# SLIDE-3D/SLIDE

Hardware: AMD Instinct MI355X
Metric: latent shapes/sec (pos+feat DDPM, 1000 steps, 16 pts) (higher is better)
Workload: dtype f16 (MFMA operands + activation storage; f32 accumulate, norm statistics, softmax); position DDPM: two-term f16 operand splits (fp32-grade); 1 GPU; BASELINE configs[1]+[2]: airplane position DDPM (16x3) + chair feature DDPM (16x51), batch 256 per GPU; 1 step = one reverse step of each; shape = 1000+1000 steps; batch_per_gpu=256, prec=fp16, pos_prec=split, replay=eager, pos_batch_multiple=2, pos_stream_cus=176, prime_steps=0, finite=True

## Files before the change

### slide_amd/csrc/gemm_ring.hip

```cpp
#include "gemm_common.h"
#include "gemm_small.h"
#include "launch.h"

namespace {

template <int PREC, int NPXL, int CBW, bool PAIRRES = false>
__global__ __launch_bounds__(256, (PREC == SLIDE_PREC_SPLIT && NPXL == 4) ? 1 : 2) void gemm_kernel(GemmArgs a) {
  using T = typename TileT<PREC>::T;
  constexpr int LDK = TileT<PREC>::LDK;
  constexpr int EPL = TileT<PREC>::EPL;
  constexpr int TPR = BK / EPL;
  constexpr int RPP = 256 / TPR;
  constexpr int TN = 32 * CBW;
  constexpr int XP = TM / RPP, WP = TN / RPP;
  extern __shared__ __attribute__((aligned(16))) unsigned char smem_raw[];
  constexpr bool SPLIT = PREC == SLIDE_PREC_SPLIT;
  using TS = typename std::conditional<SPLIT, _Float16, T>::type;
  TS *const sbase = reinterpret_cast<TS *>(smem_raw);
  constexpr int STAGE = (SPLIT ? 2 : 1) * (TM + TN) * LDK;
  constexpr int NSTG = SPLIT ? 1 : 2;
  constexpr bool AFF_LDS = PREC != SLIDE_PREC_F16 && NPXL >= 7;
  constexpr int AFF_NS = TM >> (NPXL >= 7 ? NPXL : 7);

  const int ntc = (a.n_cob + CBW - 1) / CBW;
  const int ntr = (a.rows + TM - 1) / TM;
  const int xcd = blockIdx.x & 7, q0 = blockIdx.x >> 3;
  const int tc = q0 % ntc, tr = (q0 / ntc) * 8 + xcd;
  if (tr >= ntr) return;
  const int row0 = tr * TM, cob0 = tc * CBW;
  const int tid = threadIdx.x, lane = tid & 63, wave = tid >> 6;
  const int half = lane >> 5, col = lane & 31;
  const T *X = reinterpret_cast<const T *>(a.X);
  const T *W = reinterpret_cast<const T *>(a.W);

  f32x16 acc[CBW][2];
  f32x16 acc2[SPLIT ? CBW : 1][2];
#pragma unroll
  for (int i = 0; i < CBW; ++i)
#pragma unroll
    for (int j = 0; j < 2; ++j)
#pragma unroll
      for (int r = 0; r < 16; ++r) {
        acc[i][j][r] = 0.f;
        if (SPLIT) acc2[SPLIT ? i : 0][j][r] = 0.f;
      }

  float4 xr[XP], wr[WP];
  const int l_row = tid / TPR, l_c = (tid % TPR) * EPL;

  auto load_chunk = [&](int kc) {
#pragma unroll
    for (int p = 0; p < XP; ++p) {
      const int grow = row0 + p * RPP + l_row;
      float4 v = make_float4(0.f, 0.f, 0.f, 0.f);
      if (grow < a.rows) {
        v = *reinterpret_cast<const float4 *>(X + (size_t)grow * a.x_ld + kc * BK + l_c);
        if (a.in_scale && !AFF_LDS) {
          const size_t o = (size_t)(grow >> NPXL) * a.in_bs + kc * BK + l_c;
          if (PREC != SLIDE_PREC_F16) {
            const float4 sc = *reinterpret_cast<const float4 *>(a.in_scale + o);
            const float4 sh = *reinterpret_cast<const float4 *>(a.in_shift + o);
            v.x = v.x * sc.x + sh.x; v.y = v.y * sc.y + sh.y; v.z = v.z * sc.z + sh.z; v.w = v.w * sc.w + sh.w;
          } else {
            f16x8 h = *reinterpret_cast<f16x8 *>(&v);
#pragma unroll
            for (int j = 0; j < 8; ++j) h[j] = (_Float16)((float)h[j] * a.in_scale[o + j] + a.in_shift[o + j]);
            v = *reinterpret_cast<float4 *>(&h);
          }
        }
      }
      xr[p] = v;
    }
#pragma unroll
    for (int p = 0; p < WP; ++p) {
      const int gco = cob0 * 32 + p * RPP + l_row;
      wr[p] = gco < a.n_cob * 32 ? *reinterpret_cast<const float4 *>(W + (size_t)gco * a.k_pad + kc * BK + l_c)
                                 : make_float4(0.f, 0.f, 0.f, 0.f);
    }
  };
  const float *aff_lds = nullptr;
  auto store_chunk = [&](int s, int kc) {
    TS *Xs = sbase + s * STAGE;
    TS *Ws = Xs + TM * LDK;
    if constexpr (AFF_LDS) {
      if (a.in_scale) {
#pragma unroll
        for (int p = 0; p < XP; ++p) {
          const int trow = p * RPP + l_row;
          if (row0 + trow < a.rows) {
            const float *ap = aff_lds + (size_t)((trow >> NPXL) * 2) * a.k_pad + kc * BK + l_c;
            const float4 sc = *reinterpret_cast<const float4 *>(ap), sh = *reinterpret_cast<const float4 *>(ap + a.k_pad);
            float4 &v = xr[p];
            v.x = v.x * sc.x + sh.x; v.y = v.y * sc.y + sh.y; v.z = v.z * sc.z + sh.z; v.w = v.w * sc.w + sh.w;
          }
        }
      }
    }
    if constexpr (SPLIT) {
      _Float16 *Xl = Xs + (TM + TN) * LDK, *Wl = Xl + TM * LDK;
#pragma unroll
      for (int p = 0; p < XP; ++p) {
        f16x4 hi, lo;
        split4(xr[p], hi, lo);
        *reinterpret_cast<f16x4 *>(Xs + (p * RPP + l_row) * LDK + l_c) = hi;
        *reinterpret_cast<f16x4 *>(Xl + (p * RPP + l_row) * LDK + l_c) = lo;
      }
#pragma unroll
      for (int p = 0; p < WP; ++p) {
        f16x4 hi, lo;
        split4(wr[p], hi, lo);
        *reinterpret_cast<f16x4 *>(Ws + (p * RPP + l_row) * LDK + l_c) = hi;
        *reinterpret_cast<f16x4 *>(Wl + (p * RPP + l_row) * LDK + l_c) = lo;
      }
    } else {
#pragma unroll
      for (int p = 0; p < XP; ++p) *reinterpret_cast<float4 *>(Xs + (p * RPP + l_row) * LDK + l_c) = xr[p];
#pragma unroll
      for (int p = 0; p < WP; ++p) *reinterpret_cast<float4 *>(Ws + (p * RPP + l_row) * LDK + l_c) = wr[p];
    }
  };
  auto compute = [&](int s) {
    const TS *Xs = sbase + s * STAGE;
    const TS *Ws = Xs + TM * LDK;
    if constexpr (SPLIT) {
      const _Float16 *Xl = Xs + (TM + TN) * LDK, *Wl = Xl + TM * LDK;
#pragma unroll
      for (int st = 0; st < 2; ++st) {
        f16x8 ah[CBW], al[CBW], bh[2], bl[2];
#pragma unroll
        for (int cb = 0; cb < CBW; ++cb) {
          ah[cb] = *reinterpret_cast<const f16x8 *>(Ws + (cb * 32 + col) * LDK + st * 16 + half * 8);
          al[cb] = *reinterpret_cast<const f16x8 *>(Wl + (cb * 32 + col) * LDK + st * 16 + half * 8);
        }
#pragma unroll
        for (int rb = 0; rb < 2; ++rb) {
          bh[rb] = *reinterpret_cast<const f16x8 *>(Xs + (wave * 64 + rb * 32 + col) * LDK + st * 16 + half * 8);
          bl[rb] = *reinterpret_cast<const f16x8 *>(Xl + (wave * 64 + rb * 32 + col) * LDK + st * 16 + half * 8);
        }
#pragma unroll
        for (int cb = 0; cb < CBW; ++cb)
#pragma unroll
          for (int rb = 0; rb < 2; ++rb) {
            acc[cb][rb] = __builtin_amdgcn_mfma_f32_32x32x16_f16(ah[cb], bh[rb], acc[cb][rb], 0, 0, 0);
            acc2[SPLIT ? cb : 0][rb] = __builtin_amdgcn_mfma_f32_32x32x16_f16(ah[cb], bl[rb], acc2[SPLIT ? cb : 0][rb], 0, 0, 0);
            acc2[SPLIT ? cb : 0][rb] = __builtin_amdgcn_mfma_f32_32x32x16_f16(al[cb], bh[rb], acc2[SPLIT ? cb : 0][rb], 0, 0, 0);
          }
      }
    } else if (PREC == SLIDE_PREC_F32) {
      const float *Xf = reinterpret_cast<const float *>(Xs);
      const float *Wf = reinterpret_cast<const float *>(Ws);
#pragma unroll
      for (int q = 0; q < 4; ++q) {
        float4 af[CBW], bf[2];
#pragma unroll
        for (int cb = 0; cb < CBW; ++cb)
          af[cb] = *reinterpret_cast<const float4 *>(Wf + (cb * 32 + col) * LDK + q * 8 + half * 4);
#pragma unroll
        for (int rb = 0; rb < 2; ++rb)
          bf[rb] = *reinterpret_cast<const float4 *>(Xf + (wave * 64 + rb * 32 + col) * LDK + q * 8 + half * 4);
#pragma unroll
        for (int cb = 0; cb < CBW; ++cb)
#pragma unroll
          for (int rb = 0; rb < 2; ++rb) {
            acc[cb][rb] = __builtin_amdgcn_mfma_f32_32x32x2f32(af[cb].x, bf[rb].x, acc[cb][rb], 0, 0, 0);
            acc[cb][rb] = __builtin_amdgcn_mfma_f32_32x32x2f32(af[cb].y, bf[rb].y, acc[cb][rb], 0, 0, 0);
            acc[cb][rb] = __builtin_amdgcn_mfma_f32_32x32x2f32(af[cb].z, bf[rb].z, acc[cb][rb], 0, 0, 0);
            acc[cb][rb] = __builtin_amdgcn_mfma_f32_32x32x2f32(af[cb].w, bf[rb].w, acc[cb][rb], 0, 0, 0);
          }
      }
    } else {
      const _Float16 *Xh = reinterpret_cast<const _Float16 *>(Xs);
      const _Float16 *Wh = reinterpret_cast<const _Float16 *>(Ws);
#pragma unroll
      for (int st = 0; st < 2; ++st) {
        f16x8 af[CBW], bf[2];
#pragma unroll
        for (int cb = 0; cb < CBW; ++cb)
          af[cb] = *reinterpret_cast<const f16x8 *>(Wh + (cb * 32 + col) * LDK + st * 16 + half * 8);
#pragma unroll
        for (int rb = 0; rb < 2; ++rb)
          bf[rb] = *reinterpret_cast<const f16x8 *>(Xh + (wave * 64 + rb * 32 + col) * LDK + st * 16 + half * 8);
#pragma unroll
        for (int cb = 0; cb < CBW; ++cb)
#pragma unroll
          for (int rb = 0; rb < 2; ++rb)
            acc[cb][rb] = __builtin_amdgcn_mfma_f32_32x32x16_f16(af[cb], bf[rb], acc[cb][rb], 0, 0, 0);
      }
    }
  };

  uint32_t *const epi_lds = reinterpret_cast<uint32_t *>(smem_raw + NSTG * (size_t)STAGE * sizeof(TS));
  float *const vec_lds = reinterpret_cast<float *>(epi_lds + CBW * EPI_DW + (CBW * EPI_DW) % 4);
  stage_epilogue_tables<CBW>(a, cob0, tid, epi_lds, vec_lds);
  if constexpr (AFF_LDS) {
    if (a.in_scale) {
      float *al = vec_lds + CBW * 96;
      const int nb = a.rows >> NPXL;
      for (int i = tid * 4; i < AFF_NS * a.k_pad; i += 1024) {
        const int sm = i / a.k_pad, k = i - sm * a.k_pad;
        int b = (row0 >> NPXL) + sm;
        b = b < nb ? b : nb - 1;
        *reinterpret_cast<float4 *>(al + (size_t)(sm * 2 + 0) * a.k_pad + k) = *reinterpret_cast<const float4 *>(a.in_scale + (size_t)b * a.in_bs + k);
        *reinterpret_cast<float4 *>(al + (size_t)(sm * 2 + 1) * a.k_pad + k) = *reinterpret_cast<const float4 *>(a.in_shift + (size_t)b * a.in_bs + k);
      }
      aff_lds = al;
      __syncthreads();
    }
  }

  const int nk = a.k_pad / BK;
#ifdef SLIDE_STAGGER
  const int koff = (tc * 5 + tr * 3) % nk;
#define KIDX(k) (((k) + koff) % nk)
#else
#define KIDX(k) (k)
#endif
  load_chunk(KIDX(0));
  store_chunk(0, KIDX(0));
  __syncthreads();
  for (int kc = 0; kc < nk; ++kc) {
    if (kc + 1 < nk) load_chunk(KIDX(kc + 1));
    compute(kc & (NSTG - 1));
    if (NSTG == 1) __syncthreads();
    if (kc + 1 < nk) store_chunk((kc + 1) & (NSTG - 1), KIDX(kc + 1));
    __syncthreads();
  }
#undef KIDX
  if constexpr (SPLIT) {
#pragma unroll
    for (int i = 0; i < CBW; ++i)
#pragma unroll
      for (int j = 0; j < 2; ++j)
#pragma unroll
        for (int r = 0; r < 16; ++r) acc[i][j][r] = fmaf(acc2[i][j][r], 1.f / 2048.f, acc[i][j][r]);
  }
  gemm_epilogue<SPLIT ? SLIDE_PREC_F32 : PREC, NPXL, CBW, 2, PAIRRES>(a, acc, row0, cob0, wave, half, col, epi_lds, vec_lds,
                                                                      reinterpret_cast<float *>(smem_raw));
}

template <int NPXL>
__global__ __launch_bounds__(256, 3) void gemm_split_small_kernel(GemmArgs a) {
  constexpr int LDK = TileT<SLIDE_PREC_SPLIT>::LDK;
  constexpr int TR = 64;
  constexpr int PLANE = TR * LDK;
  constexpr int STAGE = 4 * PLANE;
  extern __shared__ __attribute__((aligned(16))) unsigned char smem_raw[];
  _Float16 *const sbase = reinterpret_cast<_Float16 *>(smem_raw);
  const int ntc = (a.n_cob + 1) / 2;
  const int tc = blockIdx.x % ntc, tr = blockIdx.x / ntc;
  const int row0 = tr * TR, cob0 = tc * 2;
  const int tid = threadIdx.x, lane = tid & 63, wave = tid >> 6;
  const int half = lane >> 5, col = lane & 31;
  const int rb = wave >> 1, cb = wave & 1;
  const float *X = reinterpret_cast<const float *>(a.X);
  const float *W = reinterpret_cast<const float *>(a.W);
  f32x16 acc, acc2;
#pragma unroll
  for (int r = 0; r < 16; ++r) acc[r] = acc2[r] = 0.f;
  const int l_row = tid >> 3, l_c = (tid & 7) * 4;
  constexpr int PD = 3;
  float4 xr[PD][2], wr[PD][2];
  auto load_chunk = [&](int kc, float4 (&xr)[2], float4 (&wr)[2]) __attribute__((always_inline)) {
#pragma unroll
    for (int p = 0; p < 2; ++p) {
      const int grow = row0 + p * 32 + l_row;
      float4 v = make_float4(0.f, 0.f, 0.f, 0.f);
      if (grow < a.rows) {
        v = *reinterpret_cast<const float4 *>(X + (size_t)grow * a.x_ld + kc * BK + l_c);
      }
      xr[p] = v;
      const int gco = cob0 * 32 + p * 32 + l_row;
      wr[p] = gco < a.n_cob * 32 ? *reinterpret_cast<const float4 *>(W + (size_t)gco * a.k_pad + kc * BK + l_c)
                                 : make_float4(0.f, 0.f, 0.f, 0.f);
    }
  };
  const float *aff_lds = nullptr;
  auto store_chunk = [&](int s, int kc, const float4 (&xr)[2], const float4 (&wr)[2]) __attribute__((always_inline)) {
    _Float16 *Xh = sbase + s * STAGE, *Wh = Xh + PLANE, *Xl = Wh + PLANE, *Wl = Xl + PLANE;
#pragma unroll
    for (int p = 0; p < 2; ++p) {
      f16x4 hi, lo;
      float4 v = xr[p];
      if (aff_lds && row0 + p * 32 + l_row < a.rows) {
        const float *ap = aff_lds + (size_t)(((p * 32 + l_row) >> NPXL) * 2) * a.k_pad + kc * BK + l_c;
        const float4 sc = *reinterpret_cast<const float4 *>(ap), sh = *reinterpret_cast<const float4 *>(ap + a.k_pad);
        v.x = v.x * sc.x + sh.x; v.y = v.y * sc.y + sh.y; v.z = v.z * sc.z + sh.z; v.w = v.w * sc.w + sh.w;
      }
      split4(v, hi, lo);
      *reinterpret_cast<f16x4 *>(Xh + (p * 32 + l_row) * LDK + l_c) = hi;
      *reinterpret_cast<f16x4 *>(Xl + (p * 32 + l_row) * LDK + l_c) = lo;
      split4(wr[p], hi, lo);
      *reinterpret_cast<f16x4 *>(Wh + (p * 32 + l_row) * LDK + l_c) = hi;
      *reinterpret_cast<f16x4 *>(Wl + (p * 32 + l_row) * LDK + l_c) = lo;
    }
  };
  uint32_t *const epi_lds = reinterpret_cast<uint32_t *>(smem_raw + 2 * (size_t)STAGE * sizeof(_Float16));
  float *const vec_lds = reinterpret_cast<float *>(epi_lds + 2 * EPI_DW + (2 * EPI_DW) % 4);
  SLIDE_STAMP(a, 0);
  stage_epilogue_tables<2>(a, cob0, tid, epi_lds, vec_lds);
  if (a.in_scale) {
    float *al = vec_lds + 2 * 96;
    const int nb = a.rows >> NPXL;
    for (int i = tid * 4; i < (TR >> NPXL) * a.k_pad; i += 1024) {
      const int sm = i / a.k_pad, k = i - sm * a.k_pad;
      int b = (row0 >> NPXL) + sm;
      b = b < nb ? b : nb - 1;
      *reinterpret_cast<float4 *>(al + (size_t)(sm * 2 + 0) * a.k_pad + k) = *reinterpret_cast<const float4 *>(a.in_scale + (size_t)b * a.in_bs + k);
      *reinterpret_cast<float4 *>(al + (size_t)(sm * 2 + 1) * a.k_pad + k) = *reinterpret_cast<const float4 *>(a.in_shift + (size_t)b * a.in_bs + k);
    }
    aff_lds = al;
    __syncthreads();
  }
  const int nk = a.k_pad / BK;
  load_chunk(0, xr[0], wr[0]);
  store_chunk(0, 0, xr[0], wr[0]);
#pragma unroll
  for (int j = 0; j < PD; ++j)
    if (j + 1 < nk) load_chunk(j + 1, xr[j], wr[j]);
  __syncthreads();
  SLIDE_STAMP(a, 1);
  for (int kc0 = 0; kc0 < nk; kc0 += PD) {
#pragma unroll
    for (int j = 0; j < PD; ++j) {
      const int kc = kc0 + j;
      if (kc >= nk) break;
      const _Float16 *Xh = sbase + (kc & 1) * STAGE, *Wh = Xh + PLANE, *Xl = Wh + PLANE, *Wl = Xl + PLANE;
#pragma unroll
      for (int st = 0; st < 2; ++st) {
        const f16x8 ah = *reinterpret_cast<const f16x8 *>(Wh + (cb * 32 + col) * LDK + st * 16 + half * 8);
        const f16x8 al = *reinterpret_cast<const f16x8 *>(Wl + (cb * 32 + col) * LDK + st * 16 + half * 8);
        const f16x8 bh = *reinterpret_cast<const f16x8 *>(Xh + (rb * 32 + col) * LDK + st * 16 + half * 8);
        const f16x8 bl = *reinterpret_cast<const f16x8 *>(Xl + (rb * 32 + col) * LDK + st * 16 + half * 8);
        acc = __builtin_amdgcn_mfma_f32_32x32x16_f16(ah, bh, acc, 0, 0, 0);
        acc2 = __builtin_amdgcn_mfma_f32_32x32x16_f16(ah, bl, acc2, 0, 0, 0);
        acc2 = __builtin_amdgcn_mfma_f32_32x32x16_f16(al, bh, acc2, 0, 0, 0);
      }
      if (kc + 1 < nk) store_chunk((kc + 1) & 1, kc + 1, xr[j], wr[j]);
      __syncthreads();
      if (kc + 1 + PD < nk) load_chunk(kc + 1 + PD, xr[j], wr[j]);
    }
  }
  f32x16 one[1][1];
#pragma unroll
  for (int r = 0; r < 16; ++r) one[0][0][r] = fmaf(acc2[r], 1.f / 2048.f, acc[r]);
  SLIDE_STAMP(a, 2);
  gemm_epilogue<SLIDE_PREC_F32, NPXL, 1, 1>(a, one, row0 + rb * 32, cob0 + cb, 0, half, col, epi_lds + cb * EPI_DW, vec_lds + cb * 96,
                                            nullptr);
  SLIDE_STAMP(a, 5);
#ifdef SLIDE_TIMELINE
  if (a.dbg) { asm volatile("s_waitcnt vmcnt(0)" ::: "memory"); SLIDE_STAMP(a, 6); }
#endif
}

template <int NPXL, int CBW, int NST, int BKT, bool AFF, int WC = 1, bool GAT = false, bool PAIRRES = false, bool ATTN = false>
__device__ __forceinline__ void glds_tile(const GemmArgs &a, unsigned char *smem_raw, const int tr, const int tc) {
  using T = _Float16;
  constexpr int NW = 4 * WC, NT = 256 * WC;
  constexpr int TN = 32 * CBW * WC;
  constexpr int TNS = ((TM + TN + 16 * NW - 1) / (16 * NW)) * (16 * NW) - TM;
  constexpr int RT = TM + TNS;
  constexpr int ROWB = BKT * 2;
  constexpr int PPR = ROWB / 16;
  constexpr int RPI = 64 / PPR;
  constexpr int NI = RT / RPI;
  constexpr int LPW = NI / NW;
  constexpr int STAGE_B = RT * ROWB;
  constexpr int SWS = BKT == 32 ? 2 : 1;
  static_assert(NI % NW == 0, "tile rows must split evenly over the waves");
  static_assert(!AFF || WC == 1, "the affine variant is four-wave only");

  const int row0 = tr * TM, cob0 = tc * CBW * WC;
  const int tid = threadIdx.x, lane = tid & 63, wv = tid >> 6, wave = wv & 3, wc = wv >> 2;
  const int half = lane >> 5, col = lane & 31;

  SLIDE_STAMP(a, 0);
  constexpr int NXI = TM / (RPI * NW);
  static_assert(TM % (RPI * NW) == 0, "X rows must fill whole DMA instructions");
  const size_t x_cs = (BKT == 32 && a.x_ld == 32) ? (size_t)a.rows * 32 : BKT;
  const size_t w_cs = (BKT == 32 && a.w_cm) ? (size_t)a.n_cob * 32 * 32 : BKT;
  const int w_ld = (BKT == 32 && a.w_cm) ? 32 : a.k_pad;
  const size_t g_cs = (GAT && BKT == 32 && a.g_ldf == 32) ? (size_t)(a.rows >> NPXL) * 16 * 32 : BKT;
  const T *gp[LPW];
  const T *ga[GAT ? LPW : 1];
#pragma unroll
  for (int j = 0; j < LPW; ++j) {
    const int trow = RPI * (j * NW + wv) + lane / PPR;
    const int piece = (lane % PPR) ^ ((trow >> SWS) & (PPR - 1));
    if (trow < TM) {
      int grow = row0 + trow;
      grow = grow < a.rows ? grow : a.rows - 1;
      gp[j] = reinterpret_cast<const T *>(a.X) + (size_t)grow * a.x_ld + piece * 8;
      if (GAT) {
        const int smp = grow >> NPXL, pxl = grow & ((1 << NPXL) - 1);
        const int nb = a.gidx[(smp * 16 + (pxl >> a.g_klog2)) * 16 + (pxl & ((1 << a.g_klog2) - 1))];
        ga[j] = reinterpret_cast<const T *>(a.gfeat) + (size_t)(smp * 16 + nb) * a.g_ldf + piece * 8;
        gp[j] -= (size_t)a.g_nsplit * x_cs;
      }
    } else {
      int gco = cob0 * 32 + (trow - TM);
      gco = gco < a.n_cob * 32 ? gco : a.n_cob * 32 - 1;
      gp[j] = reinterpret_cast<const T *>(a.W) + (size_t)gco * w_ld + piece * 8;
      if (GAT) ga[j] = gp[j];
    }
  }
  auto issue = [&](int kc, int st) {
#pragma unroll
    for (int j = 0; j < LPW; ++j) {
      const T *src = (j < NXI) ? ((GAT && kc < a.g_nsplit) ? ga[GAT ? j : 0] + (size_t)kc * g_cs : gp[j] + (size_t)kc * x_cs)
                               : gp[j] + (size_t)kc * w_cs;
      __builtin_amdgcn_global_load_lds((const GLOBAL_AS void *)src,
                                       (__attribute__((address_space(3))) void *)(smem_raw + (size_t)st * STAGE_B +
                                                                                  (j * NW + wv) * 1024),
                                       16, 0, 0);
    }
  };

  const int nk = a.k_pad / BKT;
#pragma unroll
  for (int s0 = 0; s0 < NST - 1; ++s0)
    if (s0 < nk) issue(s0, s0);
  uint32_t *const epi_lds = reinterpret_cast<uint32_t *>(smem_raw + (size_t)NST * STAGE_B);
  float *const vec_lds = reinterpret_cast<float *>(epi_lds + CBW * WC * EPI_DW + (CBW * WC * EPI_DW) % 4);
  stage_epilogue_tables<CBW * WC, NT>(a, cob0, tid, epi_lds, vec_lds);
  constexpr int NSAMP = (1 << NPXL) >= TM ? 1 : TM >> NPXL;
  _Float16 *const aff_lds = reinterpret_cast<_Float16 *>(vec_lds + CBW * WC * 96);
  if (AFF) {
    static_assert(!AFF || NPXL >= 6, "the affine variant assumes one sample per wave");
    const int tps = a.aff_tps > 1 ? a.aff_tps : 1;
    const int nb = (a.rows >> NPXL) / tps, n_aff = NSAMP * a.k_pad;
    for (int i0 = tid; i0 < n_aff; i0 += 1024) {
      float sc4[4], sh4[4], ad4[4];
#pragma unroll
      for (int u = 0; u < 4; ++u) {
        const int i = i0 + 256 * u < n_aff ? i0 + 256 * u : i0;
        const int sm = i / a.k_pad, k = i - sm * a.k_pad;
        int b = ((row0 >> NPXL) + sm) / tps;
        b = b < nb ? b : nb - 1;
        sc4[u] = a.in_scale[(size_t)b * a.in_bs + k];
        sh4[u] = a.in_shift[(size_t)b * a.in_bs + k];
        ad4[u] = (a.in_add && k < a.add_n) ? a.in_add[(size_t)b * a.add_bs + k] : 0.f;
      }
#pragma unroll
      for (int u = 0; u < 4; ++u) {
        const int i = i0 + 256 * u;
        if (i >= n_aff) break;
        const int sm = i / a.k_pad, k = i - sm * a.k_pad;
        aff_lds[(sm * 3 + 0) * a.k_pad + k] = (_Float16)sc4[u];
        aff_lds[(sm * 3 + 1) * a.k_pad + k] = (_Float16)sh4[u];
        aff_lds[(sm * 3 + 2) * a.k_pad + k] = (_Float16)ad4[u];
      }
    }
  }
  const _Float16 *const aff_w = aff_lds + (size_t)((wave * 64) >> NPXL) * 3 * a.k_pad;
  const bool aff_relu = AFF && a.aff_relu;
  const bool aff_add = AFF && a.in_add && a.add_n > 0;

  f32x16 acc[CBW][2];
#pragma unroll
  for (int i = 0; i < CBW; ++i)
#pragma unroll
    for (int j = 0; j < 2; ++j)
#pragma unroll
      for (int r = 0; r < 16; ++r) acc[i][j][r] = 0.f;

  int wrow[CBW], wkey[CBW], xrow[2], xkey[2];
#pragma unroll
  for (int cb = 0; cb < CBW; ++cb) {
    const int trow = TM + (wc * CBW + cb) * 32 + col;
    wrow[cb] = trow * ROWB; wkey[cb] = (trow >> SWS) & (PPR - 1);
  }
#pragma unroll
  for (int rb = 0; rb < 2; ++rb) {
    const int trow = wave * 64 + rb * 32 + col;
    xrow[rb] = trow * ROWB; xkey[rb] = (trow >> SWS) & (PPR - 1);
  }

  SLIDE_STAMP(a, 1);
  for (int kc = 0; kc < nk; ++kc) {
    if (kc + NST - 2 < nk) asm volatile("s_waitcnt vmcnt(%0)" ::"n"((NST - 2) * LPW) : "memory");
    else asm volatile("s_waitcnt vmcnt(0)" ::: "memory");
    __builtin_amdgcn_s_barrier();
    if (kc + NST - 1 < nk) issue(kc + NST - 1, (kc + NST - 1) % NST);
    const unsigned char *sb = smem_raw + (size_t)(kc % NST) * STAGE_B;
#pragma unroll
    for (int st2 = 0; st2 < BKT / 16; ++st2) {
      f16x8 af[CBW], bf[2];
      const int piece = st2 * 2 + half;
#pragma unroll
      for (int cb = 0; cb < CBW; ++cb) af[cb] = *reinterpret_cast<const f16x8 *>(sb + wrow[cb] + ((piece ^ wkey[cb]) << 4));
#pragma unroll
      for (int rb = 0; rb < 2; ++rb) bf[rb] = *reinterpret_cast<const f16x8 *>(sb + xrow[rb] + ((piece ^ xkey[rb]) << 4));
      if (AFF) {
        const f16x8 sc = *reinterpret_cast<const f16x8 *>(aff_w + kc * BKT + piece * 8);
        const f16x8 sh = *reinterpret_cast<const f16x8 *>(aff_w + a.k_pad + kc * BKT + piece * 8);
#pragma unroll
        for (int rb = 0; rb < 2; ++rb) bf[rb] = __builtin_elementwise_fma(bf[rb], sc, sh);
        if (aff_relu || aff_add) {
          const f16x8 ad = *reinterpret_cast<const f16x8 *>(aff_w + 2 * a.k_pad + kc * BKT + piece * 8);
          const f16x8 zero = {0, 0, 0, 0, 0, 0, 0, 0};
#pragma unroll
          for (int rb = 0; rb < 2; ++rb) bf[rb] = (aff_relu ? __builtin_elementwise_max(bf[rb], zero) : bf[rb]) + ad;
        }
      }
#pragma unroll
      for (int cb = 0; cb < CBW; ++cb)
#pragma unroll
        for (int rb = 0; rb < 2; ++rb)
          acc[cb][rb] = __builtin_amdgcn_mfma_f32_32x32x16_f16(af[cb], bf[rb], acc[cb][rb], 0, 0, 0);
    }
  }
  __syncthreads();
  SLIDE_STAMP(a, 2);

  if constexpr (ATTN)
    attend_epilogue<CBW>(a, acc, row0, cob0, wave, half, col, vec_lds, reinterpret_cast<float *>(smem_raw));
  else
    gemm_epilogue<SLIDE_PREC_F16, NPXL, CBW, 2, PAIRRES>(a, acc, row0, cob0 + wc * CBW, wave, half, col, epi_lds + wc * CBW * EPI_DW,
                                             vec_lds + wc * CBW * 96,
                                             reinterpret_cast<float *>(smem_raw) + wc * (256 + 128) * CBW);
  SLIDE_STAMP(a, 5);
#ifdef SLIDE_TIMELINE
  if (a.dbg) {
    asm volatile("s_waitcnt vmcnt(0)" ::: "memory");
    SLIDE_STAMP(a, 6);
  }
#endif
}

template <int NPXL, int CBW, int NST, int BKT, bool AFF, bool GAT = false, bool PAIRRES = false>
__global__ __launch_bounds__(256, 2) void gemm_glds_kernel(GemmArgs a) {
  extern __shared__ __attribute__((aligned(16))) unsigned char smem_raw[];
  const int ntc = (a.n_cob + CBW - 1) / CBW;
  const int ntr = (a.rows + TM - 1) / TM;
  const int xcd = blockIdx.x & 7;
  if (!a.sched) {
    const int q0 = blockIdx.x >> 3;
    const int tc = q0 % ntc, tr = (q0 / ntc) * 8 + xcd;
    if (tr >= ntr) return;
    glds_tile<NPXL, CBW, NST, BKT, AFF, 1, GAT, PAIRRES>(a, smem_raw, tr, tc);
    return;
  }
  const int my_tiles = ((ntr - xcd + 7) / 8) * ntc;
  volatile int *const s_tile = reinterpret_cast<volatile int *>(smem_raw + a.shm_bytes - 16);
  const bool fixed = a.stagger < 0;
  int next = blockIdx.x >> 3;
  const int step = gridDim.x >> 3;
  if (a.stagger > 0 && threadIdx.x < 64) {
    const unsigned slot = __builtin_amdgcn_s_getreg((3 << 11) | (0 << 6) | 4);
    if (slot & 1) {
      const unsigned long long t0 = wall_clock64();
      while (wall_clock64() - t0 < (unsigned long long)a.stagger) __builtin_amdgcn_s_sleep(32);
    }
  }
  for (;;) {
    int t = next;
    next += step;
    if (!fixed) {
      if (threadIdx.x == 0) *s_tile = atomicAdd(&a.sched[xcd], 1);
      __syncthreads();
      t = __builtin_amdgcn_readfirstlane(*s_tile);
    }
    if (t >= my_tiles) break;
#ifdef SLIDE_TIMELINE
    GemmArgs a2 = a;
    if (a.dbg) a2.dbg = a.dbg + ((long long)(xcd + 8 * t) - (long long)blockIdx.x) * 16;
    glds_tile<NPXL, CBW, NST, BKT, AFF, 1, GAT, PAIRRES>(a2, smem_raw, (t / ntc) * 8 + xcd, t % ntc);
#else
    glds_tile<NPXL, CBW, NST, BKT, AFF, 1, GAT, PAIRRES>(a, smem_raw, (t / ntc) * 8 + xcd, t % ntc);
#endif
    __syncthreads();
  }
  if (!fixed && threadIdx.x == 0 && atomicAdd(&a.sched[8], 1) == (int)gridDim.x - 1) {
#pragma unroll
    for (int x = 0; x < 9; ++x) a.sched[x] = 0;
  }
}

template <int NPXL, bool AFF, bool GAT, bool PAIRRES = false>
__global__ __launch_bounds__(256, 3) void gemm_glds_occ3_kernel(GemmArgs a) {
  extern __shared__ __attribute__((aligned(16))) unsigned char smem_raw[];
  const int ntc = (a.n_cob + 1) / 2;
  const int ntr = (a.rows + TM - 1) / TM;
  const int xcd = blockIdx.x & 7, q0 = blockIdx.x >> 3;
  const int tc = q0 % ntc, tr = (q0 / ntc) * 8 + xcd;
  if (tr >= ntr) return;
  glds_tile<NPXL, 2, 2, 32, AFF, 1, GAT, PAIRRES>(a, smem_raw, tr, tc);
}

template <bool AFF>
__global__ __launch_bounds__(256, 3) void gemm_attend_kernel(GemmArgs a) {
  extern __shared__ __attribute__((aligned(16))) unsigned char smem_raw[];
  const int ntc = (a.n_cob + 1) / 2;
  const int ntr = (a.rows + TM - 1) / TM;
  const int xcd = blockIdx.x & 7, q0 = blockIdx.x >> 3;
  const int tc = q0 % ntc, tr = (q0 / ntc) * 8 + xcd;
  if (tr >= ntr) return;
  glds_tile<8, 2, 2, 32, AFF, 1, false, false, true>(a, smem_raw, tr, tc);
}

template <int NPXL, int CBW, int NST>
__global__ __launch_bounds__(512, 2) void gemm_glds8_kernel(GemmArgs a) {
  extern __shared__ __attribute__((aligned(16))) unsigned char smem_raw[];
  const int ntc = (a.n_cob + 2 * CBW - 1) / (2 * CBW);
  const int ntr = (a.rows + TM - 1) / TM;
  const int xcd = blockIdx.x & 7, q0 = blockIdx.x >> 3;
  const int tc = q0 % ntc, tr = (q0 / ntc) * 8 + xcd;
  if (tr >= ntr) return;
  glds_tile<NPXL, CBW, NST, 32, false, 2>(a, smem_raw, tr, tc);
}

template <int NST, bool AFF>
__global__ __launch_bounds__(256, 3) void gemm_small_kernel(GemmArgs a) {
  small_body<NST, AFF, 0>(a, PairArgs(), blockIdx.x);
}

template <bool FP>
__global__ __launch_bounds__(256, 3) void pair_first_kernel(GemmArgs a, PairArgs pa) {
  small_body<2, false, FP ? 2 : 1>(a, pa, blockIdx.x);
}

template <int PREC, int NPXL, int CBW, bool PAIRRES = false>
// ... 295 lines not shown
```

### slide_amd/csrc/pair_norm.h

```cpp
#pragma once
#include "gemm_common.h"

namespace {

template <bool FP, typename TT, int NT>
__device__ __forceinline__ void pair_norm2_body(int ld, const float *__restrict__ y, const float *__restrict__ xyz,
                                                const float *__restrict__ wa, const float *__restrict__ wb,
                                                const SlideEpi *__restrict__ epi, TT *__restrict__ ta,
                                                TT *__restrict__ tb, const int *__restrict__ nbr,
                                                const float *__restrict__ d2t, const float *__restrict__ wt,
                                                const float *__restrict__ vv_in, float *__restrict__ vv_out,
                                                const SlideGnFin *__restrict__ finp, const int b, const int nthr, float *dyn_l) {
  __shared__ float sx[48];
  __shared__ int sq[16 * 8];
  __shared__ float sd[16 * 8], sw[16 * 8];
  __shared__ float csum[2048], csq[2048];
  __shared__ float grp[32][2];
  const int tid = threadIdx.x;
  if (tid < 48) sx[tid] = xyz[(size_t)b * 48 + tid];
  if (FP)
    for (int t = tid; t < 128; t += nthr) {
      const int slot = (b * 16 + (t >> 3)) * 16 + (t & 7);
      sq[t] = nbr[slot]; sd[t] = d2t[slot]; sw[t] = wt[slot];
    }
  SlideGnFin f = {};
  if (finp) {
    f = *finp;
    for (int c = tid; c < f.C; c += nthr) {
      csum[c] = f.sum[(size_t)b * f.bs + c];
      csq[c] = f.sq[(size_t)b * f.bs + c];
    }
  }
  __syncthreads();
  for (int c = tid; c < ld; c += nthr) {
    const SlideEpi e = epi[c >> 5];
    const int cl = c & 31;
    float av[16], bv[16];
    const float4 ca = *reinterpret_cast<const float4 *>(wa + (size_t)c * 4), cb = *reinterpret_cast<const float4 *>(wb + (size_t)c * 4);
#pragma unroll
    for (int p = 0; p < 16; ++p) {
      const float x0 = sx[p * 3], x1 = sx[p * 3 + 1], x2 = sx[p * 3 + 2];
      av[p] = y[((size_t)b * 16 + p) * ld + c] + (ca.x * x0 + ca.y * x1 + ca.z * x2);
      bv[p] = cb.x * x0 + cb.y * x1 + cb.z * x2;
    }
    float vd = 0.f, vw = 0.f;
    if (FP) { vd = vv_in[c]; vw = vv_in[ld + c]; }
    float g = 1.f, sh = 0.f;
    if (e.mode != SLIDE_EPI_RAW) {
      const bool pre_relu = (e.flags & SLIDE_F_PRE_RELU) != 0;
      float s = 0.f, ss = 0.f;
      if (!FP && !pre_relu) {
        float A = 0.f, Bs = 0.f, A2 = 0.f, B2 = 0.f;
#pragma unroll
        for (int p = 0; p < 16; ++p) { A += av[p]; Bs += bv[p]; A2 = fmaf(av[p], av[p], A2); B2 = fmaf(bv[p], bv[p], B2); }
        s = 16.f * (A + Bs);
        ss = fmaf(2.f * A, Bs, 16.f * (A2 + B2));
      } else if (!FP) {
#pragma unroll
        for (int p = 0; p < 16; ++p)
#pragma unroll
          for (int q = 0; q < 16; ++q) {
            const float v = fmaxf(av[q] + bv[p], 0.f);
            s += v; ss = fmaf(v, v, ss);
          }
      } else {
#pragma unroll
        for (int p = 0; p < 16; ++p) dyn_l[p * (NT + 1) + tid] = av[p];
#pragma unroll
        for (int p = 0; p < 16; ++p)
#pragma unroll
          for (int j = 0; j < 8; ++j) {
            const int sl = p * 8 + j;
            float v = dyn_l[sq[sl] * (NT + 1) + tid] + bv[p] + sd[sl] * vd + sw[sl] * vw;
            if (pre_relu) v = fmaxf(v, 0.f);
            s += v; ss = fmaf(v, v, ss);
          }
      }
      if (e.mode == SLIDE_EPI_STATS) {
        if (finp) {
          const int idx = (int)(e.stats_sum - f.sum) + cl;
          csum[idx] = s * e.stats_scale;
          csq[idx] = ss * e.stats_scale;
        } else {
          e.stats_sum[(size_t)b * e.stats_bs + cl] = s * e.stats_scale;
          e.stats_sq[(size_t)b * e.stats_bs + cl] = ss * e.stats_scale;
        }
      } else {
        for (int m = 1; m < e.gs; m <<= 1) {
          s += __shfl_xor(s, m, 64);
          ss += __shfl_xor(ss, m, 64);
        }
        const float mean = s * e.inv_count;
        const float var = fmaxf(ss * e.inv_count - mean * mean, 0.f);
        g = e.gamma[cl] * __builtin_amdgcn_rsqf(var + GN_EPS);
        sh = e.beta[cl] - mean * g;
        if (cl >= e.n_norm) { g = 1.f; sh = 0.f; }
      }
    }
#pragma unroll
    for (int p = 0; p < 16; ++p) {
      ta[((size_t)b * 16 + p) * ld + c] = (TT)(av[p] * g + sh);
      tb[((size_t)b * 16 + p) * ld + c] = (TT)(bv[p] * g);
    }
    if (FP) {
      vv_out[(size_t)b * 2 * ld + c] = vd * g;
      vv_out[(size_t)b * 2 * ld + ld + c] = vw * g;
    }
  }
  if (!finp) return;
  __syncthreads();
  if (tid < 32) {
    float mean = 0.f, rstd = 0.f;
    if (tid < f.G) {
      float S = 0.f, SS = 0.f;
      const int c_end = f.gend[tid];
      for (int c = f.gstart[tid]; c < c_end; ++c) { S += csum[c]; SS += csq[c]; }
      mean = S * f.inv_count;
      const float var = fmaxf(SS * f.inv_count - mean * mean, 0.f);
      rstd = 1.0f / sqrtf(var + GN_EPS);
    }
    grp[tid][0] = mean; grp[tid][1] = rstd;
  }
  __syncthreads();
  for (int c = tid; c < f.C; c += nthr) {
    const int g = f.gid[c];
    float sc = 1.f, sh = 0.f;
    if (g >= 0) {
      sc = f.gamma[c] * grp[g][1];
      sh = f.beta[c] - grp[g][0] * sc;
    }
    f.scale[(size_t)b * f.bs + c] = sc;
    f.shift[(size_t)b * f.bs + c] = sh;
  }
}

template <bool FP, typename TT = _Float16, int NT = 1024>
__global__ __launch_bounds__(NT) void pair_norm2_kernel(int ld, const float *__restrict__ y, const float *__restrict__ xyz,
                                                          const float *__restrict__ wa, const float *__restrict__ wb,
                                                          const SlideEpi *__restrict__ epi, TT *__restrict__ ta,
                                                          TT *__restrict__ tb, const int *__restrict__ nbr,
                                                          const float *__restrict__ d2t, const float *__restrict__ wt,
                                                          const float *__restrict__ vv_in, float *__restrict__ vv_out,
                                                          const SlideGnFin *__restrict__ finp) {
  extern __shared__ __attribute__((aligned(16))) float dyn_l[];
  pair_norm2_body<FP, TT, NT>(ld, y, xyz, wa, wb, epi, ta, tb, nbr, d2t, wt, vv_in, vv_out, finp, blockIdx.x, blockDim.x, dyn_l);
}

}
```

Measured before the change: 431.4 shapes/s.

## Hoist global loads ahead of LDS staging in ring GEMM and pair-norm kernels

In the ring GEMM, the first K-chunk loads and the prefetch loads are now issued before the epilogue tables and affine LDS are staged, so global latency overlaps that setup. In pair_norm2, the per-block inputs are loaded into registers before the first barrier, and the per-channel y/wa/wb/vv loads are issued up front. Those inputs are xyz, neighbour tables, epilogue descriptors (copied into a compact LDS struct), group-norm finalise params and the channel sums. The non-FP path also fixes the FMA contraction order, and the output stores use byte-offset addressing. This trades more registers and code complexity for fewer serialised global-latency stalls ahead of the barriers.

Measured after the change: 432.9 shapes/s (median of 6 runs). No clear change (+0.3%).

```diff
diff --git a/slide_amd/csrc/gemm_ring.hip b/slide_amd/csrc/gemm_ring.hip
--- a/slide_amd/csrc/gemm_ring.hip
+++ b/slide_amd/csrc/gemm_ring.hip
@@ -297,6 +297,12 @@
   uint32_t *const epi_lds = reinterpret_cast<uint32_t *>(smem_raw + 2 * (size_t)STAGE * sizeof(_Float16));
   float *const vec_lds = reinterpret_cast<float *>(epi_lds + 2 * EPI_DW + (2 * EPI_DW) % 4);
   SLIDE_STAMP(a, 0);
+  const int nk = a.k_pad / BK;
+  float4 xr0[2], wr0[2];
+  load_chunk(0, xr0, wr0);
+#pragma unroll
+  for (int j = 0; j < PD; ++j)
+    if (j + 1 < nk) load_chunk(j + 1, xr[j], wr[j]);
   stage_epilogue_tables<2>(a, cob0, tid, epi_lds, vec_lds);
   if (a.in_scale) {
     float *al = vec_lds + 2 * 96;
@@ -311,12 +317,7 @@
     aff_lds = al;
     __syncthreads();
   }
-  const int nk = a.k_pad / BK;
-  load_chunk(0, xr[0], wr[0]);
-  store_chunk(0, 0, xr[0], wr[0]);
-#pragma unroll
-  for (int j = 0; j < PD; ++j)
-    if (j + 1 < nk) load_chunk(j + 1, xr[j], wr[j]);
+  store_chunk(0, 0, xr0, wr0);
   __syncthreads();
   SLIDE_STAMP(a, 1);
   for (int kc0 = 0; kc0 < nk; kc0 += PD) {
diff --git a/slide_amd/csrc/pair_norm.h b/slide_amd/csrc/pair_norm.h
--- a/slide_amd/csrc/pair_norm.h
+++ b/slide_amd/csrc/pair_norm.h
@@ -2,6 +2,16 @@
 #include "gemm_common.h"
 
 namespace {
+
+__device__ __forceinline__ float pair_b16(const float4 cb, const float x0, const float x1, const float x2, const bool lead_x0) {
+#pragma clang fp contract(off)
+  const float t = lead_x0 ? fmaf(cb.x, x0, cb.y * x1) : fmaf(cb.y, x1, cb.x * x0);
+  return t + cb.z * x2;
+}
+__device__ __forceinline__ float pair_a16(const float y, const float4 ca, const float x0, const float x1, const float x2) {
+#pragma clang fp contract(off)
+  return y + fmaf(ca.z, x2, fmaf(ca.y, x1, ca.x * x0));
+}
 
 template <bool FP, typename TT, int NT>
 __device__ __forceinline__ void pair_norm2_body(int ld, const float *__restrict__ y, const float *__restrict__ xyz,
@@ -16,35 +26,94 @@
   __shared__ float sd[16 * 8], sw[16 * 8];
   __shared__ float csum[2048], csq[2048];
   __shared__ float grp[32][2];
+  struct EpiL {
+    int mode, flags, gs, n_norm, stats_bs, soff;
+    float inv_count, stats_scale;
+    const float *gamma, *beta;
+    float *stats_sum, *stats_sq;
+  };
+  __shared__ EpiL sepi[64];
   const int tid = threadIdx.x;
-  if (tid < 48) sx[tid] = xyz[(size_t)b * 48 + tid];
-  if (FP)
-    for (int t = tid; t < 128; t += nthr) {
+  SlideGnFin f = {};
+  if (finp) f = *finp;
+  const float sx_r = xyz[(size_t)b * 48 + (tid < 48 ? tid : 47)];
+  int sq_r[2] = {0, 0};
+  float sd_r[2] = {0.f, 0.f}, sw_r[2] = {0.f, 0.f};
+  if (FP) {
+#pragma unroll
+    for (int u = 0; u < 2; ++u) {
+      const int t = tid + u * nthr < 128 ? tid + u * nthr : 127;
       const int slot = (b * 16 + (t >> 3)) * 16 + (t & 7);
-      sq[t] = nbr[slot]; sd[t] = d2t[slot]; sw[t] = wt[slot];
-    }
-  SlideGnFin f = {};
+      sq_r[u] = nbr[slot]; sd_r[u] = d2t[slot]; sw_r[u] = wt[slot];
+    }
+  }
+  const int nblk = ld >> 5;
+  EpiL el;
+  {
+    const SlideEpi &e = epi[tid < nblk ? tid : nblk - 1];
+    el.mode = e.mode; el.flags = e.flags; el.gs = e.gs; el.n_norm = e.n_norm; el.stats_bs = e.stats_bs;
+    el.inv_count = e.inv_count; el.stats_scale = e.stats_scale;
+    el.gamma = e.gamma; el.beta = e.beta; el.stats_sum = e.stats_sum; el.stats_sq = e.stats_sq;
+  }
+  float4 ca, cb;
+  float yv[16], vd_n = 0.f, vw_n = 0.f;
+  auto request = [&](int c) __attribute__((always_inline)) {
+    ca = *reinterpret_cast<const float4 *>(wa + (size_t)c * 4);
+    cb = *reinterpret_cast<const float4 *>(wb + (size_t)c * 4);
+    const unsigned co = (unsigned)c * 4u;
+#pragma unroll
+    for (int p = 0; p < 16; ++p)
+      yv[p] = *reinterpret_cast<const float *>(reinterpret_cast<const char *>(y + ((size_t)b * 16 + p) * ld) + co);
+    if (FP) { vd_n = vv_in[c]; vw_n = vv_in[ld + c]; }
+  };
+  request(tid < ld ? tid : ld - 1);
+  int gs_r = 0, ge_r = 0, fg_r[2] = {-1, -1};
+  float fga_r[2] = {0.f, 0.f}, fbe_r[2] = {0.f, 0.f};
   if (finp) {
-    f = *finp;
-    for (int c = tid; c < f.C; c += nthr) {
-      csum[c] = f.sum[(size_t)b * f.bs + c];
-      csq[c] = f.sq[(size_t)b * f.bs + c];
-    }
+    const int gi = tid < f.G ? tid : (f.G > 0 ? f.G - 1 : 0);
+    gs_r = f.gstart[gi]; ge_r = f.gend[gi];
+#pragma unroll
+    for (int u = 0; u < 2; ++u) {
+      const int c = tid + u * nthr < f.C ? tid + u * nthr : (f.C > 0 ? f.C - 1 : 0);
+      fg_r[u] = f.gid[c]; fga_r[u] = f.gamma[c]; fbe_r[u] = f.beta[c];
+    }
+    for (int c = tid; c < f.C; c += 2 * nthr) {
+      const int c1 = c + nthr < f.C ? c + nthr : c;
+      const float s0 = f.sum[(size_t)b * f.bs + c], q0 = f.sq[(size_t)b * f.bs + c];
+      const float s1 = f.sum[(size_t)b * f.bs + c1], q1 = f.sq[(size_t)b * f.bs + c1];
+      csum[c] = s0; csq[c] = q0;
+      csum[c1] = s1; csq[c1] = q1;
+    }
+  }
+  if (tid < 48) sx[tid] = sx_r;
+  if (FP) {
+#pragma unroll
+    for (int u = 0; u < 2; ++u)
+      if (tid + u * nthr < 128) { sq[tid + u * nthr] = sq_r[u]; sd[tid + u * nthr] = sd_r[u]; sw[tid + u * nthr] = sw_r[u]; }
+  }
+  if (tid < nblk) {
+    el.soff = (finp && el.mode == SLIDE_EPI_STATS) ? (int)(el.stats_sum - f.sum) : 0;
+    sepi[tid] = el;
   }
   __syncthreads();
-  for (int c = tid; c < ld; c += nthr) {
-    const SlideEpi e = epi[c >> 5];
+  auto pass = [&](const int c) __attribute__((always_inline)) {
+    const EpiL &e = sepi[c >> 5];
     const int cl = c & 31;
+    float gam_r = 0.f, bet_r = 0.f;
+    if (e.mode == SLIDE_EPI_NORM) { gam_r = e.gamma[cl]; bet_r = e.beta[cl]; }
     float av[16], bv[16];
-    const float4 ca = *reinterpret_cast<const float4 *>(wa + (size_t)c * 4), cb = *reinterpret_cast<const float4 *>(wb + (size_t)c * 4);
 #pragma unroll
     for (int p = 0; p < 16; ++p) {
       const float x0 = sx[p * 3], x1 = sx[p * 3 + 1], x2 = sx[p * 3 + 2];
-      av[p] = y[((size_t)b * 16 + p) * ld + c] + (ca.x * x0 + ca.y * x1 + ca.z * x2);
-      bv[p] = cb.x * x0 + cb.y * x1 + cb.z * x2;
-    }
-    float vd = 0.f, vw = 0.f;
-    if (FP) { vd = vv_in[c]; vw = vv_in[ld + c]; }
+      if (FP) {
+        av[p] = yv[p] + (ca.x * x0 + ca.y * x1 + ca.z * x2);
+        bv[p] = cb.x * x0 + cb.y * x1 + cb.z * x2;
+      } else {
+        av[p] = pair_a16(yv[p], ca, x0, x1, x2);
+        bv[p] = pair_b16(cb, x0, x1, x2, p < 6);
+      }
+    }
+    const float vd = vd_n, vw = vw_n;
     float g = 1.f, sh = 0.f;
     if (e.mode != SLIDE_EPI_RAW) {
       const bool pre_relu = (e.flags & SLIDE_F_PRE_RELU) != 0;
@@ -78,7 +147,7 @@
       }
       if (e.mode == SLIDE_EPI_STATS) {
         if (finp) {
-          const int idx = (int)(e.stats_sum - f.sum) + cl;
+          const int idx = e.soff + cl;
           csum[idx] = s * e.stats_scale;
           csq[idx] = ss * e.stats_scale;
         } else {
@@ -91,21 +160,28 @@
           ss += __shfl_xor(ss, m, 64);
         }
         const float mean = s * e.inv_count;
-        const float var = fmaxf(ss * e.inv_count - mean * mean, 0.f);
-        g = e.gamma[cl] * __builtin_amdgcn_rsqf(var + GN_EPS);
-        sh = e.beta[cl] - mean * g;
+        const float var = fmaxf(fmaf(-mean, mean, ss * e.inv_count), 0.f);
+        g = gam_r * __builtin_amdgcn_rsqf(var + GN_EPS);
+        sh = fmaf(-mean, g, bet_r);
         if (cl >= e.n_norm) { g = 1.f; sh = 0.f; }
       }
     }
+    const unsigned co = (unsigned)c * (unsigned)sizeof(TT);
 #pragma unroll
     for (int p = 0; p < 16; ++p) {
-      ta[((size_t)b * 16 + p) * ld + c] = (TT)(av[p] * g + sh);
-      tb[((size_t)b * 16 + p) * ld + c] = (TT)(bv[p] * g);
+      *reinterpret_cast<TT *>(reinterpret_cast<char *>(ta + ((size_t)b * 16 + p) * ld) + co) = (TT)fmaf(av[p], g, sh);
+      *reinterpret_cast<TT *>(reinterpret_cast<char *>(tb + ((size_t)b * 16 + p) * ld) + co) = (TT)(bv[p] * g);
     }
     if (FP) {
       vv_out[(size_t)b * 2 * ld + c] = vd * g;
       vv_out[(size_t)b * 2 * ld + ld + c] = vw * g;
     }
+  };
+  if (tid < ld) pass(tid);
+  for (int c = tid + nthr; c < ld; c += nthr) {
+    asm volatile("" ::: "memory");
+    request(c);
+    pass(c);
   }
   if (!finp) return;
   __syncthreads();
@@ -113,8 +189,7 @@
     float mean = 0.f, rstd = 0.f;
     if (tid < f.G) {
       float S = 0.f, SS = 0.f;
-      const int c_end = f.gend[tid];
-      for (int c = f.gstart[tid]; c < c_end; ++c) { S += csum[c]; SS += csq[c]; }
+      for (int c = gs_r; c < ge_r; ++c) { S += csum[c]; SS += csq[c]; }
       mean = S * f.inv_count;
       const float var = fmaxf(SS * f.inv_count - mean * mean, 0.f);
       rstd = 1.0f / sqrtf(var + GN_EPS);
@@ -122,16 +197,18 @@
     grp[tid][0] = mean; grp[tid][1] = rstd;
   }
   __syncthreads();
-  for (int c = tid; c < f.C; c += nthr) {
-    const int g = f.gid[c];
+  auto finalise = [&](int c, int g, float gam, float bet) __attribute__((always_inline)) {
     float sc = 1.f, sh = 0.f;
     if (g >= 0) {
-      sc = f.gamma[c] * grp[g][1];
-      sh = f.beta[c] - grp[g][0] * sc;
+      sc = gam * grp[g][1];
+      sh = bet - grp[g][0] * sc;
     }
     f.scale[(size_t)b * f.bs + c] = sc;
     f.shift[(size_t)b * f.bs + c] = sh;
-  }
+  };
+  if (tid < f.C) finalise(tid, fg_r[0], fga_r[0], fbe_r[0]);
+  if (tid + nthr < f.C) finalise(tid + nthr, fg_r[1], fga_r[1], fbe_r[1]);
+  for (int c = tid + 2 * nthr; c < f.C; c += nthr) finalise(c, f.gid[c], f.gamma[c], f.beta[c]);
 }
 
 template <bool FP, typename TT = _Float16, int NT = 1024>
```
